# vladiant/CascadeClassifier

Hardware: AMD Instinct MI355X
Metric: detection Mwindows/sec (1080p, haarcascade_frontalface) + achieved HBM GB/s (higher is better)
Workload: dtype i32+f32 (f64 stage sums)

## Files before the change

### cascadeclassifier_amd/csrc/cc_detect.hip

```cpp
#include <hip/hip_runtime.h>

#include <algorithm>
#include <chrono>
#include <cmath>
#include <cstdlib>
#include <cstring>
#include <functional>
#include <sstream>
#include <future>
#include <memory>
#include <thread>

#include <dlfcn.h>
#include <sys/stat.h>
#include <unistd.h>

#include <atomic>
#include <map>
#include <mutex>
#include <unordered_set>

#include "cc_internal.h"

namespace ccamd {
// ... 729 lines not shown
  }
};

}

using namespace ccamd;

constexpr int kStageSlots = 3;

struct SpecCode {
  std::vector<char> code;
  int only_step = 0;
  int tile_y = TILE_Y;
};

struct cc_detector {
  Cascade m;
  unsigned long long serial = 0;
  int device = 0;
  int max_batch = 1;
  int pass_capacity = 1;
  hipStream_t own_stream = nullptr, stream = nullptr;
  DevBuf<int> d_stage_ntrees, d_stage_first;
  DevBuf<int> d_group_first;
  int n_groups = 0;
  int dense_from = 0x7fffffff;
  DevBuf<float> d_stage_thr;
  int wave_below = 0;
  int last_call_graph = 0;
  int stop_after = -1;
  int split_stumps = 0;
  DevBuf<HaarStumpDev> d_haar1, d_haar2;
  DevBuf<HaarStumpDev> d_haar1w, d_haar2w;
  DevBuf<HaarStumpDev> d_haar_g;
  DevBuf<LbpStumpDev> d_lbp_g, d_lbp16;
  int lbp16_all = 0;
  DevBuf<LbpStumpDev> d_lbp1, d_lbp2;
  DevBuf<HaarNodeDev> d_hnode1, d_hnode2;
  DevBuf<LbpNodeDev> d_lnode1, d_lnode2;
  DevBuf<int> d_tree_root, d_tree_leaf0;
  DevBuf<float> d_leaves;
  size_t lds = 0;
  size_t lds_spec = 0;
  size_t lds_extra = 0;
  int spec_tmode = 0;
  int spec_tile_y = TILE_Y;
  DevBuf<HaarStumpP16> d_haar_p16, d_haar_p16w;
  std::vector<std::unique_ptr<Plan>> plans;
  DevBuf<uint8_t> d_frames, d_pyr;
  DevBuf<int32_t> d_integ[2], d_hbuf, d_diag, d_tseg;
  hipStream_t front_stream = nullptr;
  hipEvent_t front_done[2] = {nullptr, nullptr}, eval_done[2] = {nullptr, nullptr}, batch_begin = nullptr;
  bool eval_pending[2] = {false, false};
  int overlap_front = 1;
  hipModule_t spec_mod = nullptr;
  hipFunction_t spec_fn = nullptr;
  hipModule_t spec_mod1 = nullptr;
  hipFunction_t spec_fn1 = nullptr;
  size_t lds_spec1 = 0;
  int spec_tile_y1 = TILE_Y;
  int last_stamp_tiles = 0;
  int spec_only_step = 0;
  int spec_stages = 0;
  std::thread spec_thread;
  std::atomic<int> spec_bg_state{0};
  std::vector<SpecCode> spec_bg_code;
  int spec_bg_stages = 0;
  int spec_bg_tmode = 0;
  std::string spec_bg_error;
  DevBuf<unsigned long long> d_masks[2];
  DevBuf<CandRaw> d_cands[2];
  DevBuf<CandOut> d_out[2];
  DevBuf<int> d_counts[2];
  int* h_counts = nullptr;
  uint8_t* h_frame = nullptr;
  size_t h_frame_bytes = 0;
  uint8_t* h_stage = nullptr;
  size_t h_stage_bytes = 0;
  int stage_slot = 0;
  int use_graph = 1;
// ... 121 lines not shown
    const int fi = m.stump_feature[i];
    d.nrect = 2;
    for (int j = 0; j < 3; j++) {
      const int32_t* r = &m.haar_rects[(size_t)fi * 12 + j * 4];
      const float wt = m.haar_weights[(size_t)fi * 3 + j];
      d.w[j] = wt;
      const bool used = j < 2 || wt != 0.0f;
      if (j == 2 && wt != 0.0f) d.nrect = 3;
      const int x = used ? r[0] : 0, y = used ? r[1] : 0, rw = used ? r[2] : 0, rh = used ? r[3] : 0;
      if (!m.haar_tilted[fi]) {
        d.ofs[j][0] = at(y, x);
        d.ofs[j][1] = at(y, x + rw);
        d.ofs[j][2] = at(y + rh, x);
        d.ofs[j][3] = at(y + rh, x + rw);
      } else {
        d.ofs[j][0] = tilt_shift + at(y, x);
        d.ofs[j][1] = tilt_shift + at(y + rh, x - rh);
        d.ofs[j][2] = tilt_shift + at(y + rw, x + rw);
        d.ofs[j][3] = tilt_shift + at(y + rw + rh, x + rw - rh);
      }
    }
    d.thr = m.stump_threshold[i];
    d.left = m.stump_left[i];
    d.right = m.stump_right[i];
    d.pad = (int)i;
  }
}
template <int STEP>
static void build_haar_stumps(const Cascade& m, std::vector<HaarStumpDev>& out) {
  const TileGeom<STEP> G(m.win_w, m.win_h);
  build_haar_stumps_at(m, out, [&](int y, int x) { return G.at(y, x); }, tile_words_padded(G.words()));
}
static int window_xy(int y, int x) { return (y << 16) | x; }
static void build_haar_gstumps(const Cascade& m, std::vector<HaarStumpDev>& out) { build_haar_stumps_at(m, out, window_xy, 0); }

struct SpecStump {
  std::string loads;
  std::string decls;
  std::string compute;
  double base = 0.;
  long long base_q = 0;
};

static const char* spec_stage_inline_attr() {
  const char* e = std::getenv("CCAMD_SPEC_NOINLINE");
  return (e && std::atoi(e) != 0) ? "__noinline__" : "__forceinline__";
}

static int spec_prefetch_depth(int d = 2) {
  if (const char* e = std::getenv("CCAMD_SPEC_PREFETCH")) d = std::max(0, std::min(4, std::atoi(e)));
  return d;
}

static void spec_emit_stage(std::string& o, const std::vector<SpecStump>& st, int depth, bool parts, const std::vector<std::string>& accs,
                            bool fixed_point = false) {
  const int nt = (int)st.size();
  static const char* kSB = "      __builtin_amdgcn_sched_barrier(0);\n";
  for (const SpecStump& t : st) o += "      " + t.decls + "\n";
  const int P = parts ? SPEC_PARTS : 1;
  char buf[128];
  int prev_nonempty = -1;
  for (int k = 0; k < P; k++) {
    const int e0 = (int)((long long)k * nt / P), e1 = (int)((long long)(k + 1) * nt / P);
    if (e0 == e1) continue;
    if (parts)
      snprintf(buf, sizeof(buf), "      if (p_lo > %d && p_lo <= %d) {\n", prev_nonempty, k);
    else
// ... 29 lines not shown
    }
    o += "      }\n";
  }
}

static std::string spec_stage_source_lbp(const Cascade& m, int n_stages, bool tile16);
template <int STEP>
static void build_lbp_stumps(const Cascade& m, std::vector<LbpStumpDev>& out);
static void build_lbp_stumps16(const Cascade& m, std::vector<LbpStumpDev>& out);

enum { TILE_32 = 0, TILE_16 = 1, TILE_PAIR16 = 2 };

static bool fits16(long long area) { return 255LL * area <= 65535LL; }

static std::vector<std::array<int, 4>> pieces16(int x, int y, int w, int h) {
  std::vector<std::array<int, 4>> out;
  const bool along_x = w >= h;
  const int len = along_x ? w : h;
  for (int k = 1; k <= std::max(len, 1); k++) {
    out.clear();
    bool ok = true;
    for (int i = 0; i < k; i++) {
      const int a = (int)((long long)i * len / k), b = (int)((long long)(i + 1) * len / k);
      if (a == b) continue;
      const std::array<int, 4> pc = along_x ? std::array<int, 4>{x + a, y, b - a, h} : std::array<int, 4>{x, y + a, w, b - a};
      ok = ok && fits16((long long)pc[2] * pc[3]);
      out.push_back(pc);
    }
    if (ok) return out;
  }
  return {};
}

static bool tile16_eligible(const Cascade& m, int n_stages) {
  if (m.max_nodes_per_tree > 1) return false;
  const int total = (int)m.stage_ntrees.size();
  n_stages = std::min<int>(n_stages, total);
  const char* on = std::getenv("CCAMD_SPEC_TILE16");
  if (on ? std::atoi(on) == 0 : !(m.feature_type == CC_FEATURE_LBP && n_stages == total)) return false;
  if (m.feature_type == CC_FEATURE_HAAR) {
    if (m.has_tilted) return false;
    const int nrx = m.win_w - 2, nry = m.win_h - 2;
    if (nrx < 2 || !fits16((long long)(nrx - (nrx >> 1)) * nry)) return false;
    if (!fits16(std::max(m.win_w, m.win_h))) return false;
    return true;
  }
  for (int s = 0; s < n_stages; s++)
    for (int i = 0; i < m.stage_ntrees[(size_t)s]; i++) {
      const int32_t* r = &m.lbp_rects[(size_t)m.stump_feature[(size_t)m.stage_first[(size_t)s] + i] * 4];
      if (!fits16((long long)r[2] * r[3])) return false;
    }
  return true;
}

static bool build_haar_stumps_p16(const Cascade& m, std::vector<HaarStumpP16>& out) {
  const TileGeomP G(m.win_w, m.win_h);
  out.assign(m.stump_feature.size(), HaarStumpP16{});
  for (size_t i = 0; i < out.size(); i++) {
    HaarStumpP16& d = out[i];
    std::memset(&d, 0, sizeof(d));
    const int fi = m.stump_feature[i];
    if (m.haar_tilted[(size_t)fi]) return false;
    d.nrect = 2;
    int np = 0;
    for (int j = 0; j < 3; j++) {
      const int32_t* r = &m.haar_rects[(size_t)fi * 12 + j * 4];
      const float wt = m.haar_weights[(size_t)fi * 3 + j];
      d.w[j] = wt;
      const bool used = j < 2 || wt != 0.0f;
      if (j == 2 && wt != 0.0f) d.nrect = 3;
      if (!used || r[2] <= 0 || r[3] <= 0) continue;
      const auto pcs = pieces16(r[0], r[1], r[2], r[3]);
      if (pcs.empty()) return false;
      for (const auto& pc : pcs) {
        if (np >= P16_PIECES) return false;
        const int o4[4] = {G.at(pc[1], pc[0]), G.at(pc[1], pc[0] + pc[2]), G.at(pc[1] + pc[3], pc[0]), G.at(pc[1] + pc[3], pc[0] + pc[2])};
        for (int k = 0; k < 4; k++) {
          if (o4[k] < 0 || o4[k] > 65535) return false;
// ... 1049 lines not shown
    };
    EvalLaunch launches[2];
    int n_launches = 0;
    const bool run_spec = d->spec_fn && d->m.max_nodes_per_tree <= 1;
    if (run_spec) {
      const int want[2][2] = {{d->spec_tile_y, d->spec_only_step}, {d->spec_fn1 ? d->spec_tile_y1 : 0, 1}};
      for (int i = 0; i < 2; i++) {
        if (want[i][0] == 0) continue;
        EvalLaunch L{i == 0 ? d->spec_fn : d->spec_fn1, i == 0 ? d->lds_spec : d->lds_spec1, P->n_tiles, P->d_tiles.p};
        if (!(want[i][0] == TILE_Y && want[i][1] == 0)) {
          const auto it = P->other_tiles.find(tile_list_key(want[i][0], want[i][1]));
          if (it == P->other_tiles.end() || !it->second)
            return set_error(CC_ERR_HIP, "internal: no tile list for tiles of %d window rows (step %d)", want[i][0], want[i][1]);
          L.n_tiles = it->second->n;
          L.tiles = it->second->d.p;
        }
        launches[n_launches++] = L;
      }
    } else
      launches[n_launches++] = EvalLaunch{nullptr, d->lds, P->n_tiles, P->d_tiles.p};
    size_t stamp_tiles = 0;
    for (int i = 0; i < n_launches; i++) stamp_tiles += (size_t)launches[i].n_tiles;
    if (std::getenv("CCAMD_DEBUG_STAMPS")) {
      CC_HIP(d->d_stamps.ensure(std::max<size_t>(stamp_tiles * (size_t)nf * STAMP_SLOTS, 1)));
      CC_HIP(hipMemsetAsync(d->d_stamps.p, 0, stamp_tiles * (size_t)nf * STAMP_SLOTS * sizeof(unsigned long long), st));
      A.stamps = d->d_stamps.p;
    }
    A.dbg_codes = debug ? d->d_dbg_codes.p : nullptr;
    A.dbg_sums = debug ? d->d_dbg_sums.p : nullptr;
    A.stumps1 = haar ? (const void*)d->d_haar1.p : (const void*)d->d_lbp1.p;
    A.stumps2 = haar ? (const void*)d->d_haar2.p : (const void*)d->d_lbp2.p;
    A.wstumps1 = d->d_haar1w.p ? (const void*)d->d_haar1w.p : A.stumps1;
    A.wstumps2 = d->d_haar2w.p ? (const void*)d->d_haar2w.p : A.stumps2;
    A.gstumps = haar ? (const void*)d->d_haar_g.p : (const void*)d->d_lbp_g.p;
    A.lbp16_all = d->lbp16_all;
    if (!haar && d->d_lbp16.p) A.wstumps2 = d->d_lbp16.p;
    if (d->spec_fn && d->spec_tmode == TILE_PAIR16) {
      A.gstumps = d->d_haar_p16.p;
      A.wstumps2 = d->d_haar_p16w.p;
    }
    A.trees = d->m.max_nodes_per_tree > 1 ? 1 : 0;
    A.nodes1 = haar ? (const void*)d->d_hnode1.p : (const void*)d->d_lnode1.p;
    A.nodes2 = haar ? (const void*)d->d_hnode2.p : (const void*)d->d_lnode2.p;
    A.tree_root = d->d_tree_root.p;
    A.tree_leaf0 = d->d_tree_leaf0.p;
    A.leaves = d->d_leaves.p;
    for (int i = 0; i < n_launches; i++) {
      const EvalLaunch& L = launches[i];
      if (L.n_tiles == 0) continue;
      A.tiles = L.tiles;
      if (L.fn) {
        void* params[] = {&A};
        EvScope ev1(d, i == 1 ? EV_EVAL_STEP1 : -1, st);
        CC_HIP(hipModuleLaunchKernel(L.fn, (unsigned)L.n_tiles, (unsigned)nf, 1, EVAL_THREADS, 1, 1, (unsigned)L.lds, st, params, nullptr));
      } else if (haar)
        hipLaunchKernelGGL(k_eval_haar, dim3(L.n_tiles, nf), dim3(EVAL_THREADS), L.lds, st, A);
      else
        hipLaunchKernelGGL(k_eval_lbp, dim3(L.n_tiles, nf), dim3(EVAL_THREADS), L.lds, st, A);
      if (A.stamps) A.stamps += (size_t)L.n_tiles * (size_t)nf * STAMP_SLOTS;
    }
    d->last_stamp_tiles = (int)stamp_tiles;
  }
  if (fs != st) {
    CC_HIP(hipEventRecord(d->eval_done[slot], st));
    d->eval_pending[slot] = true;
  }
  {
    EvScope ev(d, EV_FILTER, st);
    hipLaunchKernelGGL(k_filter_candidates, dim3(64), dim3(256), 0, st, d->d_cands[slot].p, d->d_counts[slot].p, d->cand_cap, P->d_sd.p,
                       d->d_masks[slot].p, P->mask_frame_words, d->d_out[slot].p, d->d_counts[slot].p + 1);
    if (debug && P->n_grid_rows)
      hipLaunchKernelGGL(k_debug_visited, dim3(P->n_grid_rows), dim3(256), 0, st, P->d_sd.p, ns, P->d_gridrow_first.p,
// ... 482 lines not shown
      api.lib = dlopen(name, RTLD_NOW | RTLD_LOCAL);
      if (api.lib) break;
    }
    if (!api.lib) return;
    auto sym = [&](const char* n) { return dlsym(api.lib, n); };
    api.create = reinterpret_cast<decltype(api.create)>(sym("hiprtcCreateProgram"));
    api.compile = reinterpret_cast<decltype(api.compile)>(sym("hiprtcCompileProgram"));
    api.log_size = reinterpret_cast<decltype(api.log_size)>(sym("hiprtcGetProgramLogSize"));
    api.log = reinterpret_cast<decltype(api.log)>(sym("hiprtcGetProgramLog"));
    api.code_size = reinterpret_cast<decltype(api.code_size)>(sym("hiprtcGetCodeSize"));
    api.code = reinterpret_cast<decltype(api.code)>(sym("hiprtcGetCode"));
    api.destroy = reinterpret_cast<decltype(api.destroy)>(sym("hiprtcDestroyProgram"));
    api.version = reinterpret_cast<decltype(api.version)>(sym("hiprtcVersion"));
  });
  return api;
}

static const char kSpecPrelude[] =
    "typedef signed char int8_t;\ntypedef unsigned char uint8_t;\ntypedef short int16_t;\ntypedef unsigned short uint16_t;\n"
    "typedef int int32_t;\ntypedef unsigned int uint32_t;\ntypedef long long int64_t;\ntypedef unsigned long long uint64_t;\n";

struct SpecModulePlan {
  int only_step, tile_y;
};
static std::vector<SpecModulePlan> spec_modules(const Cascade& m, int tmode) {
  auto valid = [&](int ty) { return ty >= EVAL_WAVES && ty <= 32 && ty % EVAL_WAVES == 0; };
  auto env_rows = [&](const char* name, int dflt) {
    const char* e = std::getenv(name);
    const int v = e ? std::atoi(e) : dflt;
    return valid(v) ? v : dflt;
  };
  if (tmode == TILE_PAIR16 || m.has_tilted) return {{0, TILE_Y}};
  const bool lbp16 = m.feature_type == CC_FEATURE_LBP && tmode == TILE_16;
  const bool haar32 = tmode == TILE_32 && m.feature_type == CC_FEATURE_HAAR;
  const bool rows_given = std::getenv("CCAMD_SPEC_TILE_Y") != nullptr;
  const int all = env_rows("CCAMD_SPEC_TILE_Y", lbp16 ? 20 : TILE_Y);
  const bool two = (haar32 || std::getenv("CCAMD_SPEC_TWO_MODULES")) && !std::getenv("CCAMD_SPEC_ONE_MODULE");
  if (!two) return {{0, all}};
  return {{2, env_rows("CCAMD_SPEC_TILE_Y2", all)}, {1, env_rows("CCAMD_SPEC_TILE_Y1", (haar32 && !rows_given) ? 12 : all)}};
}

static cc_status compile_specialised(const std::string& src, const std::string& arch, int n_stages, bool lbp, int tmode, int tile_y, int only_step, int win_w, int win_h, std::vector<char>& code) {
  const bool tile16 = tmode == TILE_16;
  static std::mutex mu;
  static std::map<std::string, std::vector<char>> cache;
  const std::string o_arch = "--offload-arch=" + arch, o_k = "-DCC_SPEC_STAGES=" + std::to_string(n_stages);
  const std::string o_ty = "-DCC_TILE_Y=" + std::to_string(tile_y), o_th = "-DCC_EVAL_THREADS=" + std::to_string(EVAL_THREADS);
  std::string o_w = "-DCC_EVAL_MIN_WAVES_PER_EU=" + std::to_string(tile16 ? (tile_y >= 20 ? 6 : 7) : CC_EVAL_MIN_WAVES_PER_EU);
  const std::string o_step = "-DCC_ONLY_STEP=" + std::to_string(only_step);
  if (const char* e = std::getenv("CCAMD_SPEC_WAVES_PER_EU")) o_w = "-DCC_EVAL_MIN_WAVES_PER_EU=" + std::to_string(std::max(1, std::min(8, std::atoi(e))));
  const std::string o_w0 = "-DCC_SPEC_W0=" + std::to_string(win_w), o_h0 = "-DCC_SPEC_H0=" + std::to_string(win_h);
  std::vector<const char*> optv = {o_arch.c_str(), "-O3", "-std=c++17", "-ffp-contract=off", "-fno-fast-math", o_k.c_str(), o_ty.c_str(), o_th.c_str(), o_w.c_str(), o_w0.c_str(), o_h0.c_str()};
  if (only_step) optv.push_back(o_step.c_str());
  if (lbp) optv.push_back("-DCC_SPEC_LBP");
  if (tile16) optv.push_back("-DCC_SPEC_TILE16");
  if (tmode == TILE_PAIR16) optv.push_back("-DCC_SPEC_PAIR16");
  std::vector<std::string> extra;
  if (const char* e = std::getenv("CCAMD_SPEC_EXTRA_FLAGS")) {
    std::istringstream is(e);
    for (std::string w; is >> w;) extra.push_back(w);
  }
  for (const std::string& w : extra) optv.push_back(w.c_str());
  const char* const* opts = optv.data();
  const int n_opts = (int)optv.size();
  std::string key;
  {
    int major = 0, minor = 0;
    const HipRtcApi& rtc = hiprtc_api();
    if (rtc.version) (void)rtc.version(&major, &minor);
    key += "hiprtc " + std::to_string(major) + "." + std::to_string(minor) + " ";
  }
  for (int i = 0; i < n_opts; i++) key += std::string(opts[i]) + " ";
  key += "#" + src;
  {
    std::lock_guard<std::mutex> lk(mu);
    auto it = cache.find(key);
    if (it != cache.end()) {
      code = it->second;
      return CC_OK;
    }
  }
// ... 131 lines not shown
  struct Loaded {
    hipModule_t mod = nullptr;
    hipFunction_t fn = nullptr;
    size_t lds = 0;
    int tile_y = TILE_Y, only_step = 0;
  };
  std::vector<Loaded> L;
  auto unload_all = [&]() {
    for (Loaded& x : L)
      if (x.mod) (void)hipModuleUnload(x.mod);
  };
  for (const SpecCode& c : codes) {
    Loaded x;
    x.tile_y = c.tile_y;
    x.only_step = c.only_step;
    const char* entry = c.only_step == 1 ? "k_eval_spec_step1" : c.only_step == 2 ? "k_eval_spec_step2" : "k_eval_spec";
    if (hipModuleLoadData(&x.mod, c.code.data()) != hipSuccess || hipModuleGetFunction(&x.fn, x.mod, entry) != hipSuccess) {
      (void)hipGetLastError();
      if (x.mod) (void)hipModuleUnload(x.mod);
      unload_all();
      return set_error(CC_ERR_HIP, "cc_detector_specialize: the compiled module does not load or has no entry point");
    }
    const int ty = c.tile_y;
    const int step = c.only_step ? c.only_step : debug_only_step();
    x.lds = d->lds;
    if (tmode == TILE_32) {
      const TileGeom<1> G1(d->m.win_w, d->m.win_h, ty);
      const TileGeom<2> G2(d->m.win_w, d->m.win_h, ty);
      const int words = step == 1 ? G1.words() : step == 2 ? G2.words() : std::max(G1.words(), G2.words());
      x.lds = eval_lds_bytes(words, d->m.has_tilted, haar_k, ty) + d->lds_extra;
    } else if (tmode == TILE_16) {
      const TileGeom<1> G1(d->m.win_w, d->m.win_h, ty);
      const TileGeom16 G2(d->m.win_w, d->m.win_h, ty);
      x.lds = eval_lds_bytes(std::max(G1.words(), G2.words()), false, haar_k, ty) + d->lds_extra;
    } else if (tmode == TILE_PAIR16) {
      const TileGeom<1> G1(d->m.win_w, d->m.win_h);
      const TileGeomP G2(d->m.win_w, d->m.win_h);
      x.lds = std::max(eval_lds_bytes(G1.words(), false), eval_lds_bytes_pair(G2.words())) + d->lds_extra;
      if (!d->d_haar_p16.p) {
        std::vector<HaarStumpP16> tp, tw;
        build_haar_stumps_p16(d->m, tp);
        std::vector<HaarStumpDev> geo;
        build_haar_stumps_at(d->m, geo, [&](int y, int x2) { return G2.at(y, x2); }, 0);
        const std::vector<HaarStumpDev> order = d->wave_below > 0 && !std::getenv("CCAMD_NO_WAVE_SCHEDULE") ? schedule_for_wave_phase(d->m, geo) : geo;
        tw.reserve(order.size());
        for (const HaarStumpDev& r : order) tw.push_back(tp[(size_t)r.pad]);
        CC_HIP(d->d_haar_p16.upload(tp, d->stream));
        CC_HIP(d->d_haar_p16w.upload(tw, d->stream));
        CC_HIP(hipStreamSynchronize(d->stream));
      }
    }
    if (x.lds > 64 * 1024) {
      const hipError_t e = hipFuncSetAttribute(reinterpret_cast<const void*>(x.fn), hipFuncAttributeMaxDynamicSharedMemorySize, (int)x.lds);
      if (e != hipSuccess) {
        (void)hipGetLastError();
        (void)hipModuleUnload(x.mod);
        unload_all();
        return set_error(CC_ERR_UNSUPPORTED, "cc_detector_specialize: %zu bytes of LDS per tile cannot be requested for a run-time module (%s)",
                         x.lds, hipGetErrorString(e));
      }
    }
    if (std::getenv("CCAMD_TRACE_HOST")) {
      int nb = 0;
      if (hipModuleOccupancyMaxActiveBlocksPerMultiprocessor(&nb, x.fn, EVAL_THREADS, x.lds) != hipSuccess) (void)hipGetLastError();
      std::fprintf(stderr, "[ccamd host] specialised kernel: tile mode %d, tiles of step %d (0 = all), %d window rows, %zu bytes of LDS per block, %d resident blocks per CU\n",
                   tmode, c.only_step, ty, x.lds, nb);
    }
// ... 208 lines not shown
    d->dense_from = 0x7fffffff;
    if (dense_stage >= 1)
      for (int g = (int)gf.size() - 2; g >= 1; g--)
        if (gf[(size_t)g] >= dense_stage) d->dense_from = g;
    CC_HIP(d->d_group_first.upload(gf, d->stream));
    CC_HIP(hipStreamSynchronize(d->stream));
  }
  if (trees) {
    std::vector<int> root(d->m.tree_first_node.begin(), d->m.tree_first_node.end()), leaf0(d->m.tree_first_leaf.begin(), d->m.tree_first_leaf.end());
    CC_HIP(d->d_tree_root.upload(root, d->stream));
    CC_HIP(d->d_tree_leaf0.upload(leaf0, d->stream));
    CC_HIP(d->d_leaves.upload(d->m.leaves, d->stream));
    if (haar) {
      std::vector<HaarNodeDev> n1, n2;
      build_haar_nodes<1>(d->m, n1);
      build_haar_nodes<2>(d->m, n2);
      CC_HIP(d->d_hnode1.upload(n1, d->stream));
      CC_HIP(d->d_hnode2.upload(n2, d->stream));
      CC_HIP(hipStreamSynchronize(d->stream));
    } else {
      std::vector<LbpNodeDev> n1, n2;
      build_lbp_nodes<1>(d->m, n1);
      build_lbp_nodes<2>(d->m, n2);
      CC_HIP(d->d_lnode1.upload(n1, d->stream));
      CC_HIP(d->d_lnode2.upload(n2, d->stream));
      CC_HIP(hipStreamSynchronize(d->stream));
    }
  } else if (haar) {
    std::vector<HaarStumpDev> s1, s2;
    build_haar_stumps<1>(d->m, s1);
    build_haar_stumps<2>(d->m, s2);
    CC_HIP(d->d_haar1.upload(s1, d->stream));
    CC_HIP(d->d_haar2.upload(s2, d->stream));
    std::vector<HaarStumpDev> sg;
    if (!d->m.has_tilted) build_haar_gstumps(d->m, sg);
    CC_HIP(d->d_haar_g.upload(sg, d->stream));
    CC_HIP(hipStreamSynchronize(d->stream));
    if (d->wave_below > 0 && !std::getenv("CCAMD_NO_WAVE_SCHEDULE")) {
      const std::vector<HaarStumpDev> w1 = schedule_for_wave_phase(d->m, s1), w2 = schedule_for_wave_phase(d->m, s2);
      CC_HIP(d->d_haar1w.upload(w1, d->stream));
      CC_HIP(d->d_haar2w.upload(w2, d->stream));
      CC_HIP(hipStreamSynchronize(d->stream));
    }
    CC_HIP(hipStreamSynchronize(d->stream));
  } else {
    std::vector<LbpStumpDev> s1, s2;
    build_lbp_stumps<1>(d->m, s1);
    build_lbp_stumps<2>(d->m, s2);
    CC_HIP(d->d_lbp1.upload(s1, d->stream));
    CC_HIP(d->d_lbp2.upload(s2, d->stream));
    std::vector<LbpStumpDev> sg, s16;
    build_lbp_gstumps(d->m, sg);
    CC_HIP(d->d_lbp_g.upload(sg, d->stream));
    d->lbp16_all = 1;
    for (size_t i = 0; i < d->m.stump_feature.size(); i++) {
      const int32_t* r = &d->m.lbp_rects[(size_t)d->m.stump_feature[i] * 4];
      if (!fits16((long long)r[2] * r[3])) d->lbp16_all = 0;
    }
    if (d->lbp16_all) {
      build_lbp_stumps16(d->m, s16);
      CC_HIP(d->d_lbp16.upload(s16, d->stream));
    }
    CC_HIP(hipStreamSynchronize(d->stream));
  }
  if (const char* e = std::getenv("CCAMD_AUTO_SPECIALIZE")) {
    const int k = std::atoi(e);
    if (k > 0 && d->m.max_nodes_per_tree == 1) (void)spec_start_background(d.get(), k);
  }
  *out = d.release();
// ... 867 lines not shown
```

### cascadeclassifier_amd/csrc/cc_eval_kernel.inc

```

#define CC_CONST __attribute__((address_space(4)))
template <class T>
__device__ __forceinline__ const T CC_CONST* as_const_table(const T* p) {
  return (const T CC_CONST*)p;
}
template <class T>
__device__ __forceinline__ T load_record(const T CC_CONST* p) {
  static_assert(sizeof(T) % 4 == 0, "table records are dword multiples");
  T out;
  const int CC_CONST* w = (const int CC_CONST*)p;
  int* o = reinterpret_cast<int*>(&out);
#pragma unroll
  for (unsigned i = 0; i < sizeof(T) / 4; i++) o[i] = w[i];
  return out;
}

constexpr int TILE_X = 64;
#ifndef CC_TILE_Y
#define CC_TILE_Y 8
#endif
#ifndef CC_EVAL_THREADS
#define CC_EVAL_THREADS 256
#endif
#ifndef CC_EVAL_MIN_WAVES_PER_EU
// ... 84 lines not shown
    row_stride = rs16 / 2;
  }
  __host__ __device__ int at(int r, int c) const { return r * rs16 + c; }
  __host__ __device__ int words() const { return rows * row_stride; }
};

struct TileGeomP {
  static constexpr bool k16 = false;
  int cols, rows, plane, row_stride, wrow;
  __host__ __device__ TileGeomP(int W0, int H0) {
    cols = (TILE_X - 1) * 2 + W0 + 1;
    rows = (TILE_Y - 1) * 2 + H0 + 1;
    plane = ((cols + 3) / 4 * 4) / 2;
    row_stride = 2 * plane;
    for (;; row_stride += 2) {
      const int k = (2 * row_stride + 1) & 31;
      if (k == 21 || k == 25 || k == 9 || k == 13 || k == 5) break;
    }
    wrow = 2 * row_stride + 1;
  }
  __host__ __device__ int at(int r, int c) const { return r * row_stride + (r >> 1) + (c & 1) * plane + (c >> 1); }
  __host__ __device__ int words() const { return rows * row_stride + (rows >> 1) + 2; }
};

constexpr int P16_PIECES = 6;
struct HaarStumpP16 {
  unsigned short ofs[P16_PIECES][4];
  float w[3];
  float thr, left, right;
  unsigned char rect_of[P16_PIECES];
  unsigned char npieces, nrect;
};
static_assert(sizeof(HaarStumpP16) == 80, "HaarStumpP16 is loaded dword by dword");

constexpr int TILE_WINDOWS = TILE_X * TILE_Y;
constexpr int MAX_STAGES = 64;
constexpr int PART_DOUBLES = (EVAL_WAVES - 1) * 64;
constexpr int QUEUE_ROWS = TILE_WINDOWS / 32;
constexpr int VNF_PITCH = TILE_X + 32;
__host__ __device__ inline int tile_words_padded(int tile_words) { return (tile_words + 3) & ~3; }
__host__ __device__ inline size_t eval_lds_bytes(int tile_words, bool tilted, bool haar = true, int tile_y = TILE_Y) {
  return (size_t)tile_words_padded(tile_words) * 4 * (tilted ? 2 : 1) + PART_DOUBLES * 8 + (haar ? tile_y * VNF_PITCH * 4 : 0) +
         2 * (tile_y * TILE_X) * 2 + 3 * 32 * 4;
}
constexpr int PAIR_PART = EVAL_THREADS / 2;
__host__ __device__ inline size_t eval_lds_bytes_pair(int tile_words) {
  return eval_lds_bytes(tile_words, false) - PART_DOUBLES * 8 + 2 * PAIR_PART * 8;
}

constexpr int STAGE_ROWS = 12;
template <int STEP, class Geom>
__device__ __forceinline__ void stage_tile(int32_t* lds, const Geom& G, const int32_t* __restrict__ sum,
                                           const ScaleDev& S, int x0, int y0) {
  const int lane = threadIdx.x & 63, wave = __builtin_amdgcn_readfirstlane(threadIdx.x >> 6);
  const int quads = (G.cols + 3) >> 2;
  const bool right_edge = x0 + quads * 4 - 1 > S.w;
  for (int q0 = 0; q0 < quads; q0 += 64) {
    const int qd = q0 + lane;
    const int c = qd * 4, gc = x0 + c;
    const bool in_tile = qd < quads;
    const bool col_ok = in_tile && gc <= S.w;
    for (int rb = wave; rb < G.rows; rb += EVAL_WAVES * STAGE_ROWS) {
      int4 v[STAGE_ROWS];
#pragma unroll
      for (int k = 0; k < STAGE_ROWS; k++) {
        const int r = rb + k * EVAL_WAVES, gr = y0 + r;
// ... 70 lines not shown
constexpr int STAMP_SLOTS = 40;

struct LdsReader {
  const int32_t* b;
  __device__ __forceinline__ int operator()(int ofs) const { return b[ofs]; }
};
struct GlobalReader {
  const int32_t* g;
  unsigned org;
  int pitch;
  __device__ __forceinline__ int operator()(int p) const { return g[org + (unsigned)((p >> 16) * pitch + (p & 0xffff))]; }
};
template <class R>
__device__ __forceinline__ double stump_vote(const R& rd, const HaarStumpDev& sp, float vnf) {
  const int r0 = rd(sp.ofs[0][0]) - rd(sp.ofs[0][1]) - rd(sp.ofs[0][2]) + rd(sp.ofs[0][3]);
  const int r1 = rd(sp.ofs[1][0]) - rd(sp.ofs[1][1]) - rd(sp.ofs[1][2]) + rd(sp.ofs[1][3]);
  float v = sp.w[0] * (float)r0 + sp.w[1] * (float)r1;
  if (sp.nrect == 3) {
    const int r2 = rd(sp.ofs[2][0]) - rd(sp.ofs[2][1]) - rd(sp.ofs[2][2]) + rd(sp.ofs[2][3]);
    v += sp.w[2] * (float)r2;
  }
  v *= vnf;
  return (double)(v < sp.thr ? sp.left : sp.right);
}
template <class R>
__device__ __forceinline__ double stump_vote(const R& rd, const HaarStumpDev CC_CONST* spp, float vnf) {
  return stump_vote(rd, load_record(spp), vnf);
}

struct Lds16Reader {
  const unsigned short* h;
  __device__ __forceinline__ int operator()(int ofs) const { return (int)h[ofs]; }
};
template <bool M16, class R>
__device__ __forceinline__ float lbp_vote_f(const R& rd, const LbpStumpDev& sp) {
  int p[16];
#pragma unroll
  for (int j = 0; j < 16; j++) p[j] = rd(sp.ofs[j]);
  auto cell = [&](int a, int b, int c2, int d) {
    const int v = p[a] - p[b] - p[c2] + p[d];
    return M16 ? (v & 0xffff) : v;
  };
  const int c = cell(5, 6, 9, 10);
  const bool b7 = cell(0, 1, 4, 5) >= c, b6 = cell(1, 2, 5, 6) >= c, b5 = cell(2, 3, 6, 7) >= c;
  const int lo = (cell(6, 7, 10, 11) >= c ? 16 : 0) | (cell(10, 11, 14, 15) >= c ? 8 : 0) | (cell(9, 10, 13, 14) >= c ? 4 : 0) |
                 (cell(8, 9, 12, 13) >= c ? 2 : 0) | (cell(4, 5, 8, 9) >= c ? 1 : 0);
  const int l0 = b5 ? sp.subset[1] : sp.subset[0], l1 = b5 ? sp.subset[3] : sp.subset[2], l2 = b5 ? sp.subset[5] : sp.subset[4],
            l3 = b5 ? sp.subset[7] : sp.subset[6];
  const int m0 = b6 ? l1 : l0, m1 = b6 ? l3 : l2;
  const unsigned w = (unsigned)(b7 ? m1 : m0);
  return ((w >> lo) & 1u) ? sp.left : sp.right;
}

template <class R>
__device__ __forceinline__ double stump_vote(const R& rd, const LbpStumpDev CC_CONST* sp, float) {
  int p[16];
#pragma unroll
  for (int j = 0; j < 16; j++) p[j] = rd(sp->ofs[j]);
  const int c = p[5] - p[6] - p[9] + p[10];
  const int lbp = (p[0] - p[1] - p[4] + p[5] >= c ? 128 : 0) | (p[1] - p[2] - p[5] + p[6] >= c ? 64 : 0) |
                  (p[2] - p[3] - p[6] + p[7] >= c ? 32 : 0) | (p[6] - p[7] - p[10] + p[11] >= c ? 16 : 0) |
                  (p[10] - p[11] - p[14] + p[15] >= c ? 8 : 0) | (p[9] - p[10] - p[13] + p[14] >= c ? 4 : 0) |
                  (p[8] - p[9] - p[12] + p[13] >= c ? 2 : 0) | (p[4] - p[5] - p[8] + p[9] >= c ? 1 : 0);
  const int word = sp->subset[lbp >> 5];
  return (double)((word & (1 << (lbp & 31))) ? sp->left : sp->right);
}
// ... 105 lines not shown
struct cc_select {
  using type = A;
};
template <class A, class B>
struct cc_select<false, A, B> {
  using type = B;
};

template <int STEP, bool HAAR, bool TREES>
__device__ __forceinline__ void eval_tile(const EvalArgs& A, int32_t* lds, const int4 T, const ScaleDev& S) {
  using Stump = typename cc_select<HAAR, HaarStumpDev, LbpStumpDev>::type;
  using Node = typename cc_select<HAAR, HaarNodeDev, LbpNodeDev>::type;
  const Node* __restrict__ nodes = reinterpret_cast<const Node*>(STEP == 2 ? A.nodes2 : A.nodes1);
#ifdef CC_SPEC_W0
  constexpr int W0 = CC_SPEC_W0, H0 = CC_SPEC_H0;
#else
  const int W0 = A.W0, H0 = A.H0;
#endif
#ifdef CC_SPEC_TILE16
  constexpr bool G16 = STEP == 2 && !TREES;
#else
  constexpr bool G16 = false;
#endif
  using Geom = typename cc_select<G16, TileGeom16, TileGeom<STEP>>::type;
  const Geom G(W0, H0);
  double* s_part = reinterpret_cast<double*>(lds + tile_words_padded(G.words()) * ((HAAR && A.tilt_chan >= 0) ? 2 : 1));
  float* s_vnf = reinterpret_cast<float*>(s_part + PART_DOUBLES);
  unsigned short* s_q = reinterpret_cast<unsigned short*>(s_vnf + (HAAR ? TILE_Y * VNF_PITCH : 0));
  int* s_cnt = reinterpret_cast<int*>(s_q + 2 * TILE_WINDOWS);
  const int frame = blockIdx.y;
  const int32_t* sum = A.integ + ((size_t)frame * A.nchan + 0) * A.int_frame_elems + S.int_ofs;
  const int lane = threadIdx.x & 63, wave = __builtin_amdgcn_readfirstlane(threadIdx.x >> 6);
  const int gx0 = T.y * TILE_X, gy0 = T.z * TILE_Y;
  const Stump CC_CONST* stumps = as_const_table(reinterpret_cast<const Stump*>(G16 ? A.gstumps : STEP == 2 ? A.stumps2 : A.stumps1));
  const int CC_CONST* stage_first = as_const_table(A.stage_first);
  const int CC_CONST* stage_ntrees = as_const_table(A.stage_ntrees);
  const float CC_CONST* stage_thr = as_const_table(A.stage_thr);
  const bool dbg = A.dbg_codes != nullptr && frame == 0;
  auto stamp = [&](int slot) {
    if (A.stamps && threadIdx.x == 0)
      A.stamps[((size_t)blockIdx.y * gridDim.x + blockIdx.x) * STAMP_SLOTS + slot] = __builtin_amdgcn_s_memtime();
  };
  stamp(0);

  unsigned sq_raw[WIN_PER_THREAD][4];
#pragma unroll
  for (int k = 0; k < WIN_PER_THREAD; k++) {
    sq_raw[k][0] = sq_raw[k][1] = sq_raw[k][2] = sq_raw[k][3] = 0;
    if (HAAR) {
      const int gx = min(gx0 + lane, S.nx - 1), gy = min(gy0 + wave * WIN_PER_THREAD + k, S.ny - 1);
      {
        const unsigned* sq = reinterpret_cast<const unsigned*>(A.integ + ((size_t)frame * A.nchan + 1) * A.int_frame_elems + S.int_ofs);
        const int nrx = W0 - 2, nry = H0 - 2;
        size_t q0;
        int dx;
        if (STEP == 2 && A.sq_compact) {
          q0 = (size_t)(gy * 2 + 1) * S.pitchI + gx;
          dx = nrx >> 1;
        } else {
          q0 = (size_t)(gy * STEP + 1) * S.pitchI + (gx * STEP + 1);
          dx = nrx;
        }
        sq_raw[k][0] = sq[q0];
        sq_raw[k][1] = sq[q0 + dx];
        sq_raw[k][2] = sq[q0 + (size_t)nry * S.pitchI];
        sq_raw[k][3] = sq[q0 + (size_t)nry * S.pitchI + dx];
      }
    }
  }
#ifdef CC_PRIO_STAGE
  __builtin_amdgcn_s_setprio(CC_PRIO_STAGE);
#endif
  stage_tile<STEP>(lds, G, sum, S, gx0 * STEP, gy0 * STEP);
  if (HAAR && A.tilt_chan >= 0)
    stage_tile<STEP>(lds + tile_words_padded(G.words()), G,
                     A.integ + ((size_t)frame * A.nchan + A.tilt_chan) * A.int_frame_elems + S.int_ofs, S, gx0 * STEP, gy0 * STEP);
  if (threadIdx.x < 3 * 32) s_cnt[threadIdx.x] = 0;
  unsigned valsq_pre[WIN_PER_THREAD];
#pragma unroll
  for (int k = 0; k < WIN_PER_THREAD; k++) valsq_pre[k] = sq_raw[k][0] - sq_raw[k][1] - sq_raw[k][2] + sq_raw[k][3];
  __syncthreads();
#ifdef CC_PRIO_STAGE
  __builtin_amdgcn_s_setprio(0);
#endif
  stamp(1);

  if (A.stop_after == -2) return;
  auto window_base = [&](int id) { return ((id >> 6) * STEP) * G.row_stride + (id & 63); };
  auto table_reader = [&](int id) {
    if constexpr (G16)
      return GlobalReader{sum, (unsigned)((gy0 + (id >> 6)) * STEP) * (unsigned)S.pitchI + (unsigned)((gx0 + (id & 63)) * STEP), S.pitchI};
    else
      return LdsReader{lds + window_base(id)};
  };
  auto report = [&](int id, int code, double last) {
    const size_t o = (size_t)S.win_ofs + (size_t)(gy0 + (id >> 6)) * S.nx + (gx0 + (id & 63));
    A.dbg_codes[o] = code;
    if (A.dbg_sums) A.dbg_sums[o] = last;
  };
  auto emit_candidate = [&](int id, double last_sum) {
    const int slot = atomicAdd(A.cand_count, 1);
    if (slot < A.cand_cap) A.cands[slot] = CandRaw{frame, T.x, gx0 + (id & 63), gy0 + (id >> 6), last_sum};
  };
  const int skew = (STEP * G.row_stride) & 31;
  auto win_class = [&](int id) { return ((id & 63) + skew * (id >> 6)) & 31; };
  auto vnf_slot = [&](int id) { return (id >> 6) * (TILE_X + skew) + (id & 63); };
  auto enqueue = [&](bool pass, int id, int g) {
    if (g >= A.dense_from) {
      const unsigned long long m = __ballot(pass);
      int first = 0;
      if (lane == 0 && m) first = atomicAdd(&s_cnt[(g % 3) * 32], __builtin_popcountll(m));
      first = __builtin_amdgcn_readfirstlane(first);
      if (pass) s_q[(g & 1) * TILE_WINDOWS + first + __builtin_amdgcn_mbcnt_hi((unsigned)(m >> 32), __builtin_amdgcn_mbcnt_lo((unsigned)m, 0))] = (unsigned short)id;
    } else if (pass) {
      const int c = win_class(id);
      const int row = atomicAdd(&s_cnt[(g % 3) * 32 + c], 1);
      s_q[(g & 1) * TILE_WINDOWS + row * 32 + c] = (unsigned short)id;
    }
  };

  const int CC_CONST* group_first = as_const_table(A.group_first);
  auto stage_sum = [&](int s, int id, const int32_t* b, float vnf, bool want) -> double {
    double acc = 0.;
    const int first = stage_first[s], nt = stage_ntrees[s];
    if constexpr (TREES) {
      for (int j = 0; j < nt; j++) {
        const int root = as_const_table(A.tree_root)[first + j], leaf0 = as_const_table(A.tree_leaf0)[first + j];
        if (want) acc += tree_vote(b, nodes, root, leaf0, A.leaves, vnf);
      }
    } else {
#ifdef CC_SPEC_STAGES
      if (s < CC_SPEC_STAGES) return spec_stage<STEP>(s, 0, SPEC_PARTS, b, vnf);
#endif
      const auto rd = table_reader(id);
      if constexpr (HAAR) {
        Stump cur = load_record(stumps + first);
        for (int j = 0; j < nt; j++) {
          const Stump nxt = load_record(stumps + first + min(j + 1, nt - 1));
          acc += stump_vote(rd, cur, vnf);
          cur = nxt;
        }
      } else {
        for (int j = 0; j < nt; j++) acc += stump_vote(rd, stumps + first + j, vnf);
      }
    }
    return acc;
  };

  if constexpr (!HAAR && !TREES && WIN_PER_THREAD > 2) {
    const int gx = gx0 + lane;
    const double thr0 = (double)stage_thr[0];
    const int nt0 = stage_ntrees[0];
#pragma unroll 1
    for (int k = 0; k < WIN_PER_THREAD; k++) {
      const int ly = wave * WIN_PER_THREAD + k;
      const int gy = gy0 + ly;
      const int id = ly * 64 + lane;
      const int32_t* b = lds + (ly * STEP) * G.row_stride + lane;
      const bool alive = gx < S.nx && gy < S.ny;
      double acc = 0.;
      if (__any(alive)) {
#ifdef CC_SPEC_STAGES
        acc = spec_stage<STEP>(0, 0, SPEC_PARTS, b, 1.f);
#else
        for (int i = 0; i < nt0; i++) acc += stump_vote(LdsReader{b}, stumps + i, 1.f);
#endif
      }
      (void)nt0;
      bool pass = alive && !(acc < thr0);
      const bool rej0 = alive && !pass;
      const unsigned long long m = __ballot(rej0);
// ... 221 lines not shown
        } else
          enqueue(alive, id, qg + 1);
      }
    }
    auto finish = [&](bool valid, int id, double acc) {
      const bool pass = valid && !(acc < thr);
      if (dbg && valid && !pass) report(id, -st, acc);
      if (last_group) {
        if (pass) {
          emit_candidate(id, acc);
          if (dbg) report(id, 1, acc);
        }
      } else
        enqueue(pass, id, qg + 1);
    };
    if (ns > 1) {
      const int slice = wave % ns, grp = wave / ns;
      const int row = (g_split + grp) * 2 + half;
      const int i = grp * 64 + lane;
      const bool valid = row < my_rows;
      const int id = valid ? q[min(row, QUEUE_ROWS - 1) * 32 + cls] : cls;
      double acc = 0.;
      if (grp < rem) {
        [[maybe_unused]] const int32_t* b = lds + window_base(id);
        const float vnf = HAAR ? s_vnf[vnf_slot(id)] : 1.f;
        [[maybe_unused]] const auto rd = table_reader(id);
        if constexpr (HAAR) {
#ifdef CC_SPEC_STAGES
          if (!TREES && st < CC_SPEC_STAGES) {
            acc = spec_stage<STEP>(st, slice * (SPEC_PARTS / ns), (slice + 1) * (SPEC_PARTS / ns), b, vnf);
          } else
#endif
          if (slice < nt) {
            Stump cur = load_record(stumps + first + slice);
            for (int j = slice; j < nt; j += ns) {
              const Stump nxt = load_record(stumps + first + min(j + ns, nt - 1));
              acc += stump_vote(rd, cur, vnf);
              cur = nxt;
            }
          }
        } else {
#ifdef CC_SPEC_STAGES
          if (!TREES && st < CC_SPEC_STAGES)
            acc = spec_stage<STEP>(st, slice * (SPEC_PARTS / ns), (slice + 1) * (SPEC_PARTS / ns), b, vnf);
          else
#endif
            for (int j = slice; j < nt; j += ns) acc += stump_vote(rd, stumps + first + j, vnf);
        }
        if (slice) s_part[(slice - 1) * (EVAL_THREADS / ns) + i] = acc;
      }
      __syncthreads();
      if (grp < rem && slice == 0) {
        for (int k = 1; k < ns; k++) acc += s_part[(k - 1) * (EVAL_THREADS / ns) + i];
        finish(valid, id, acc);
      }
    }
  }
  if (qg >= A.ngroups || n == 0) {
    stamp(STAMP_SLOTS - 1);
    return;
  }

  if constexpr (HAAR && !TREES) {
    const unsigned short* q = s_q + (qg & 1) * TILE_WINDOWS;
    const Stump* wstumps = reinterpret_cast<const Stump*>(G16 ? A.gstumps : STEP == 2 ? A.wstumps2 : A.wstumps1);
    unsigned short* my_list = reinterpret_cast<unsigned short*>(s_part) + wave * 64;
    int numbered = 0;
    for (int r0 = 0; r0 < rows; r0 += 2) {
      const int row = r0 + half;
      const bool valid = row < my_rows;
      const int id = valid ? q[row * 32 + cls] : 0;
      const unsigned long long mask = __ballot(valid);
      const int number = numbered + __builtin_amdgcn_mbcnt_hi((unsigned)(mask >> 32), __builtin_amdgcn_mbcnt_lo((unsigned)mask, 0));
      if (valid && number % EVAL_WAVES == wave) my_list[number / EVAL_WAVES] = (unsigned short)id;
      numbered += __builtin_popcountll(mask);
    }
    const int cnt = (numbered - wave + EVAL_WAVES - 1) / EVAL_WAVES;
    const int my_id = lane < cnt ? my_list[lane] : 0;
    unsigned long long alive = cnt >= 64 ? ~0ull : ((1ull << cnt) - 1ull);
    const bool w_stamps = st + 2 < 30;
    if (w_stamps) stamp(30);
    double tot = 0., last = 0.;
    int rej = 0;
    int s2 = st;
    for (; s2 < A.nstages && alive; s2++) {
      if (A.stop_after >= 0 && s2 > A.stop_after) break;
      const int first = stage_first[s2], nt = stage_ntrees[s2];
      for (int c = 0; c < nt; c += 64) {
        const int j = c + lane;
        const Stump rec = wstumps[first + min(j, nt - 1)];
        for (unsigned long long m = alive; m; m &= m - 1ull) {
          const int k = __builtin_ctzll(m);
          const int id = __builtin_amdgcn_readlane(my_id, k);
          const float vnf = s_vnf[vnf_slot(id)];
          const double part = j < nt ? stump_vote(table_reader(id), rec, vnf) : 0.;
          const double total = wave_sum_f64(part);
          if (lane == k) tot += total;
        }
      }
      const bool mine = (alive >> lane) & 1ull;
      const bool pass = mine && !(tot < (double)stage_thr[s2]);
      if (mine) {
        last = tot;
        if (!pass) rej = s2;
      }
      tot = 0.;
      alive = __ballot(pass);
      if (w_stamps && s2 - st < 8) stamp(31 + s2 - st);
    }
    const bool accepted = s2 == A.nstages && ((alive >> lane) & 1ull);
    if (lane < cnt) {
      if (accepted) emit_candidate(my_id, last);
      if (dbg && (accepted || !((alive >> lane) & 1ull))) report(my_id, accepted ? 1 : -rej, last);
    }
  }
  if constexpr (!HAAR && !TREES && EVAL_WAVES >= 4) {
    const unsigned short* q = s_q + (qg & 1) * TILE_WINDOWS;
    unsigned short* my_list = reinterpret_cast<unsigned short*>(s_part) + wave * 64;
    float* votes = reinterpret_cast<float*>(reinterpret_cast<char*>(s_part) + EVAL_WAVES * 128) + wave * 64;
    int numbered = 0;
    for (int r0 = 0; r0 < rows; r0 += 2) {
      const int row = r0 + half;
      const bool valid = row < my_rows;
// ... 566 lines not shown
```

Measured before the change: 18240.

## Use 16-bit LDS integral tile for Haar step-2 specialised evaluation

Enables the 16-bit tile mode by default for Haar cascades. It adds a compact HaarStump16 record with ushort offsets, splitting rectangles into pieces whose sums fit 16 bits and recombining them modulo 2^16. The step-2 kernel then reads the integral image from LDS as 16-bit values, where it previously read 32-bit values or went to global memory. This halves LDS per tile and allows more waves per EU, with per-module tile rows and wave counts tuned. The cost is extra piece arithmetic for rectangles that have to be split, a more complex setup, and removal of the global Haar stump path.

```diff
diff --git a/cascadeclassifier_amd/csrc/cc_detect.hip b/cascadeclassifier_amd/csrc/cc_detect.hip
--- a/cascadeclassifier_amd/csrc/cc_detect.hip
+++ b/cascadeclassifier_amd/csrc/cc_detect.hip
@@ -785,7 +785,6 @@
   int split_stumps = 0;
   DevBuf<HaarStumpDev> d_haar1, d_haar2;
   DevBuf<HaarStumpDev> d_haar1w, d_haar2w;
-  DevBuf<HaarStumpDev> d_haar_g;
   DevBuf<LbpStumpDev> d_lbp_g, d_lbp16;
   int lbp16_all = 0;
   DevBuf<LbpStumpDev> d_lbp1, d_lbp2;
@@ -799,6 +798,7 @@
   int spec_tmode = 0;
   int spec_tile_y = TILE_Y;
   DevBuf<HaarStumpP16> d_haar_p16, d_haar_p16w;
+  DevBuf<HaarStump16> d_haar16, d_haar16w;
   std::vector<std::unique_ptr<Plan>> plans;
   DevBuf<uint8_t> d_frames, d_pyr;
   DevBuf<int32_t> d_integ[2], d_hbuf, d_diag, d_tseg;
@@ -986,7 +986,6 @@
   build_haar_stumps_at(m, out, [&](int y, int x) { return G.at(y, x); }, tile_words_padded(G.words()));
 }
 static int window_xy(int y, int x) { return (y << 16) | x; }
-static void build_haar_gstumps(const Cascade& m, std::vector<HaarStumpDev>& out) { build_haar_stumps_at(m, out, window_xy, 0); }
 
 struct SpecStump {
   std::string loads;
@@ -1082,18 +1081,61 @@
   return {};
 }
 
+static bool build_haar_stumps16(const Cascade& m, std::vector<HaarStump16>& out) {
+  const TileGeom16 G(m.win_w, m.win_h);
+  out.assign(m.stump_feature.size(), HaarStump16{});
+  for (size_t i = 0; i < out.size(); i++) {
+    HaarStump16& d = out[i];
+    std::memset(&d, 0, sizeof(d));
+    const int fi = m.stump_feature[i];
+    if (m.haar_tilted[(size_t)fi]) return false;
+    d.nrect = 2;
+    int nx = 0;
+    for (int j = 0; j < 3; j++) {
+      const int32_t* r = &m.haar_rects[(size_t)fi * 12 + j * 4];
+      const float wt = m.haar_weights[(size_t)fi * 3 + j];
+      d.w[j] = wt;
+      const bool used = j < 2 || wt != 0.0f;
+      if (j == 2 && wt != 0.0f) d.nrect = 3;
+      if (!used || r[2] <= 0 || r[3] <= 0) continue;
+      const auto pcs = pieces16(r[0], r[1], r[2], r[3]);
+      if (pcs.empty()) return false;
+      for (size_t q = 0; q < pcs.size(); q++) {
+        const auto& pc = pcs[q];
+        const int slot = q == 0 ? j : 3 + nx;
+        if (q > 0) {
+          if (nx >= S16_EXTRA) return false;
+          d.xrect = (unsigned char)(d.xrect | (j << (2 * nx)));
+          nx++;
+        }
+        const int o4[4] = {G.at(pc[1], pc[0]), G.at(pc[1], pc[0] + pc[2]), G.at(pc[1] + pc[3], pc[0]), G.at(pc[1] + pc[3], pc[0] + pc[2])};
+        for (int k = 0; k < 4; k++) {
+          if (o4[k] < 0 || o4[k] > 65535) return false;
+          d.ofs[slot][k] = (unsigned short)o4[k];
+        }
+      }
+    }
+    d.nextra = (unsigned char)nx;
+    d.thr = m.stump_threshold[i];
+    d.left = m.stump_left[i];
+    d.right = m.stump_right[i];
+  }
+  return true;
+}
+
 static bool tile16_eligible(const Cascade& m, int n_stages) {
   if (m.max_nodes_per_tree > 1) return false;
   const int total = (int)m.stage_ntrees.size();
   n_stages = std::min<int>(n_stages, total);
   const char* on = std::getenv("CCAMD_SPEC_TILE16");
-  if (on ? std::atoi(on) == 0 : !(m.feature_type == CC_FEATURE_LBP && n_stages == total)) return false;
+  if (on ? std::atoi(on) == 0 : !(m.feature_type == CC_FEATURE_HAAR || n_stages == total)) return false;
   if (m.feature_type == CC_FEATURE_HAAR) {
     if (m.has_tilted) return false;
     const int nrx = m.win_w - 2, nry = m.win_h - 2;
     if (nrx < 2 || !fits16((long long)(nrx - (nrx >> 1)) * nry)) return false;
     if (!fits16(std::max(m.win_w, m.win_h))) return false;
-    return true;
+    std::vector<HaarStump16> tmp;
+    return build_haar_stumps16(m, tmp);
   }
   for (int s = 0; s < n_stages; s++)
     for (int i = 0; i < m.stage_ntrees[(size_t)s]; i++) {
@@ -2209,12 +2251,16 @@
     A.stumps2 = haar ? (const void*)d->d_haar2.p : (const void*)d->d_lbp2.p;
     A.wstumps1 = d->d_haar1w.p ? (const void*)d->d_haar1w.p : A.stumps1;
     A.wstumps2 = d->d_haar2w.p ? (const void*)d->d_haar2w.p : A.stumps2;
-    A.gstumps = haar ? (const void*)d->d_haar_g.p : (const void*)d->d_lbp_g.p;
+    A.gstumps = haar ? nullptr : (const void*)d->d_lbp_g.p;
     A.lbp16_all = d->lbp16_all;
     if (!haar && d->d_lbp16.p) A.wstumps2 = d->d_lbp16.p;
     if (d->spec_fn && d->spec_tmode == TILE_PAIR16) {
       A.gstumps = d->d_haar_p16.p;
       A.wstumps2 = d->d_haar_p16w.p;
+    }
+    if (haar && d->spec_fn && d->spec_tmode == TILE_16) {
+      A.gstumps = d->d_haar16.p;
+      A.wstumps2 = d->d_haar16w.p;
     }
     A.trees = d->m.max_nodes_per_tree > 1 ? 1 : 0;
     A.nodes1 = haar ? (const void*)d->d_hnode1.p : (const void*)d->d_lnode1.p;
@@ -2763,12 +2809,14 @@
   };
   if (tmode == TILE_PAIR16 || m.has_tilted) return {{0, TILE_Y}};
   const bool lbp16 = m.feature_type == CC_FEATURE_LBP && tmode == TILE_16;
-  const bool haar32 = tmode == TILE_32 && m.feature_type == CC_FEATURE_HAAR;
+  const bool haar = m.feature_type == CC_FEATURE_HAAR;
   const bool rows_given = std::getenv("CCAMD_SPEC_TILE_Y") != nullptr;
   const int all = env_rows("CCAMD_SPEC_TILE_Y", lbp16 ? 20 : TILE_Y);
-  const bool two = (haar32 || std::getenv("CCAMD_SPEC_TWO_MODULES")) && !std::getenv("CCAMD_SPEC_ONE_MODULE");
+  const bool two = (haar || std::getenv("CCAMD_SPEC_TWO_MODULES")) && !std::getenv("CCAMD_SPEC_ONE_MODULE");
   if (!two) return {{0, all}};
-  return {{2, env_rows("CCAMD_SPEC_TILE_Y2", all)}, {1, env_rows("CCAMD_SPEC_TILE_Y1", (haar32 && !rows_given) ? 12 : all)}};
+  const bool haar16 = haar && tmode == TILE_16;
+  return {{2, env_rows("CCAMD_SPEC_TILE_Y2", (haar16 && !rows_given) ? 12 : all)},
+          {1, env_rows("CCAMD_SPEC_TILE_Y1", (haar && !rows_given) ? 12 : all)}};
 }
 
 static cc_status compile_specialised(const std::string& src, const std::string& arch, int n_stages, bool lbp, int tmode, int tile_y, int only_step, int win_w, int win_h, std::vector<char>& code) {
@@ -2777,7 +2825,11 @@
   static std::map<std::string, std::vector<char>> cache;
   const std::string o_arch = "--offload-arch=" + arch, o_k = "-DCC_SPEC_STAGES=" + std::to_string(n_stages);
   const std::string o_ty = "-DCC_TILE_Y=" + std::to_string(tile_y), o_th = "-DCC_EVAL_THREADS=" + std::to_string(EVAL_THREADS);
-  std::string o_w = "-DCC_EVAL_MIN_WAVES_PER_EU=" + std::to_string(tile16 ? (tile_y >= 20 ? 6 : 7) : CC_EVAL_MIN_WAVES_PER_EU);
+  int waves = tile16 ? (tile_y >= 20 ? 6 : 7) : CC_EVAL_MIN_WAVES_PER_EU;
+  if (tile16 && !lbp && only_step == 1) waves = CC_EVAL_MIN_WAVES_PER_EU;
+  if (tile16 && !lbp && only_step == 2)
+    waves = std::max(1, std::min(8, (int)((160 * 1024) / eval_lds_bytes(TileGeom16(win_w, win_h, tile_y).words(), false, true, tile_y))));
+  std::string o_w = "-DCC_EVAL_MIN_WAVES_PER_EU=" + std::to_string(waves);
   const std::string o_step = "-DCC_ONLY_STEP=" + std::to_string(only_step);
   if (const char* e = std::getenv("CCAMD_SPEC_WAVES_PER_EU")) o_w = "-DCC_EVAL_MIN_WAVES_PER_EU=" + std::to_string(std::max(1, std::min(8, std::atoi(e))));
   const std::string o_w0 = "-DCC_SPEC_W0=" + std::to_string(win_w), o_h0 = "-DCC_SPEC_H0=" + std::to_string(win_h);
@@ -2975,7 +3027,37 @@
     } else if (tmode == TILE_16) {
       const TileGeom<1> G1(d->m.win_w, d->m.win_h, ty);
       const TileGeom16 G2(d->m.win_w, d->m.win_h, ty);
-      x.lds = eval_lds_bytes(std::max(G1.words(), G2.words()), false, haar_k, ty) + d->lds_extra;
+      const int words = step == 1 ? G1.words() : step == 2 ? G2.words() : std::max(G1.words(), G2.words());
+      x.lds = eval_lds_bytes(words, false, haar_k, ty) + d->lds_extra;
+      if (haar_k && !d->d_haar16.p) {
+        std::vector<HaarStump16> tp, tw;
+        if (!build_haar_stumps16(d->m, tp)) {
+          unload_all();
+          (void)hipModuleUnload(x.mod);
+          return set_error(CC_ERR_HIP, "cc_detector_specialize: a stump does not fit the 16-bit tile's record");
+        }
+        std::vector<HaarStumpDev> g0, geo;
+        build_haar_stumps_at(d->m, g0, [&](int y, int x2) { return G2.at(y, x2) >> 1; }, 0);
+        Cascade parts = d->m;
+        parts.stage_first.clear();
+        parts.stage_ntrees.clear();
+        for (size_t s = 0; s < d->m.stage_ntrees.size(); s++) {
+          const int first = d->m.stage_first[s], nt = d->m.stage_ntrees[s];
+          for (int extra = 0; extra < 2; extra++) {
+            const int f = (int)geo.size();
+            for (int i = first; i < first + nt; i++)
+              if ((tp[(size_t)i].nextra > 0) == (extra == 1)) geo.push_back(g0[(size_t)i]);
+            parts.stage_first.push_back(f);
+            parts.stage_ntrees.push_back((int)geo.size() - f);
+          }
+        }
+        const std::vector<HaarStumpDev> order = d->wave_below > 0 && !std::getenv("CCAMD_NO_WAVE_SCHEDULE") ? schedule_for_wave_phase(parts, geo) : geo;
+        tw.reserve(order.size());
+        for (const HaarStumpDev& r : order) tw.push_back(tp[(size_t)r.pad]);
+        CC_HIP(d->d_haar16.upload(tp, d->stream));
+        CC_HIP(d->d_haar16w.upload(tw, d->stream));
+        CC_HIP(hipStreamSynchronize(d->stream));
+      }
     } else if (tmode == TILE_PAIR16) {
       const TileGeom<1> G1(d->m.win_w, d->m.win_h);
       const TileGeomP G2(d->m.win_w, d->m.win_h);
@@ -3250,9 +3332,6 @@
     build_haar_stumps<2>(d->m, s2);
     CC_HIP(d->d_haar1.upload(s1, d->stream));
     CC_HIP(d->d_haar2.upload(s2, d->stream));
-    std::vector<HaarStumpDev> sg;
-    if (!d->m.has_tilted) build_haar_gstumps(d->m, sg);
-    CC_HIP(d->d_haar_g.upload(sg, d->stream));
     CC_HIP(hipStreamSynchronize(d->stream));
     if (d->wave_below > 0 && !std::getenv("CCAMD_NO_WAVE_SCHEDULE")) {
       const std::vector<HaarStumpDev> w1 = schedule_for_wave_phase(d->m, s1), w2 = schedule_for_wave_phase(d->m, s2);
diff --git a/cascadeclassifier_amd/csrc/cc_eval_kernel.inc b/cascadeclassifier_amd/csrc/cc_eval_kernel.inc
--- a/cascadeclassifier_amd/csrc/cc_eval_kernel.inc
+++ b/cascadeclassifier_amd/csrc/cc_eval_kernel.inc
@@ -140,6 +140,15 @@
   unsigned char npieces, nrect;
 };
 static_assert(sizeof(HaarStumpP16) == 80, "HaarStumpP16 is loaded dword by dword");
+
+constexpr int S16_EXTRA = P16_PIECES - 3;
+struct HaarStump16 {
+  unsigned short ofs[P16_PIECES][4];
+  float w[3];
+  float thr, left, right;
+  unsigned char nrect, nextra, xrect, pad;
+};
+static_assert(sizeof(HaarStump16) == 76, "HaarStump16 is loaded dword by dword");
 
 constexpr int TILE_WINDOWS = TILE_X * TILE_Y;
 constexpr int MAX_STAGES = 64;
@@ -276,6 +285,30 @@
   const unsigned short* h;
   __device__ __forceinline__ int operator()(int ofs) const { return (int)h[ofs]; }
 };
+__device__ __forceinline__ double stump_vote(const Lds16Reader& rd, const HaarStump16& sp, float vnf) {
+  auto piece = [&](int p) { return (rd(sp.ofs[p][0]) - rd(sp.ofs[p][1]) - rd(sp.ofs[p][2]) + rd(sp.ofs[p][3])) & 0xffff; };
+  int r0 = piece(0), r1 = piece(1), r2 = 0;
+  if (sp.nrect == 3) r2 = piece(2);
+  if (sp.nextra) {
+#pragma unroll
+    for (int i = 0; i < S16_EXTRA; i++) {
+      if (i < sp.nextra) {
+        const int v = piece(3 + i), r = (sp.xrect >> (2 * i)) & 3;
+        r0 += r == 0 ? v : 0;
+        r1 += r == 1 ? v : 0;
+        r2 += r == 2 ? v : 0;
+      }
+    }
+  }
+  float v = sp.w[0] * (float)r0 + sp.w[1] * (float)r1;
+  if (sp.nrect == 3) v += sp.w[2] * (float)r2;
+  v *= vnf;
+  return (double)(v < sp.thr ? sp.left : sp.right);
+}
+__device__ __forceinline__ double stump_vote(const Lds16Reader& rd, const HaarStump16 CC_CONST* spp, float vnf) {
+  return stump_vote(rd, load_record(spp), vnf);
+}
+
 template <bool M16, class R>
 __device__ __forceinline__ float lbp_vote_f(const R& rd, const LbpStumpDev& sp) {
   int p[16];
@@ -447,7 +480,8 @@
   const int32_t* sum = A.integ + ((size_t)frame * A.nchan + 0) * A.int_frame_elems + S.int_ofs;
   const int lane = threadIdx.x & 63, wave = __builtin_amdgcn_readfirstlane(threadIdx.x >> 6);
   const int gx0 = T.y * TILE_X, gy0 = T.z * TILE_Y;
-  const Stump CC_CONST* stumps = as_const_table(reinterpret_cast<const Stump*>(G16 ? A.gstumps : STEP == 2 ? A.stumps2 : A.stumps1));
+  using TStump = typename cc_select<HAAR && G16, HaarStump16, Stump>::type;
+  const TStump CC_CONST* stumps = as_const_table(reinterpret_cast<const TStump*>(G16 ? A.gstumps : STEP == 2 ? A.stumps2 : A.stumps1));
   const int CC_CONST* stage_first = as_const_table(A.stage_first);
   const int CC_CONST* stage_ntrees = as_const_table(A.stage_ntrees);
   const float CC_CONST* stage_thr = as_const_table(A.stage_thr);
@@ -503,7 +537,9 @@
   if (A.stop_after == -2) return;
   auto window_base = [&](int id) { return ((id >> 6) * STEP) * G.row_stride + (id & 63); };
   auto table_reader = [&](int id) {
-    if constexpr (G16)
+    if constexpr (G16 && HAAR)
+      return Lds16Reader{reinterpret_cast<const unsigned short*>(lds + window_base(id))};
+    else if constexpr (G16)
       return GlobalReader{sum, (unsigned)((gy0 + (id >> 6)) * STEP) * (unsigned)S.pitchI + (unsigned)((gx0 + (id & 63)) * STEP), S.pitchI};
     else
       return LdsReader{lds + window_base(id)};
@@ -549,9 +585,9 @@
 #endif
       const auto rd = table_reader(id);
       if constexpr (HAAR) {
-        Stump cur = load_record(stumps + first);
+        TStump cur = load_record(stumps + first);
         for (int j = 0; j < nt; j++) {
-          const Stump nxt = load_record(stumps + first + min(j + 1, nt - 1));
+          const TStump nxt = load_record(stumps + first + min(j + 1, nt - 1));
           acc += stump_vote(rd, cur, vnf);
           cur = nxt;
         }
@@ -839,9 +875,9 @@
           } else
 #endif
           if (slice < nt) {
-            Stump cur = load_record(stumps + first + slice);
+            TStump cur = load_record(stumps + first + slice);
             for (int j = slice; j < nt; j += ns) {
-              const Stump nxt = load_record(stumps + first + min(j + ns, nt - 1));
+              const TStump nxt = load_record(stumps + first + min(j + ns, nt - 1));
               acc += stump_vote(rd, cur, vnf);
               cur = nxt;
             }
@@ -870,7 +906,7 @@
 
   if constexpr (HAAR && !TREES) {
     const unsigned short* q = s_q + (qg & 1) * TILE_WINDOWS;
-    const Stump* wstumps = reinterpret_cast<const Stump*>(G16 ? A.gstumps : STEP == 2 ? A.wstumps2 : A.wstumps1);
+    const TStump* wstumps = reinterpret_cast<const TStump*>(STEP == 2 ? A.wstumps2 : A.wstumps1);
     unsigned short* my_list = reinterpret_cast<unsigned short*>(s_part) + wave * 64;
     int numbered = 0;
     for (int r0 = 0; r0 < rows; r0 += 2) {
@@ -895,7 +931,7 @@
       const int first = stage_first[s2], nt = stage_ntrees[s2];
       for (int c = 0; c < nt; c += 64) {
         const int j = c + lane;
-        const Stump rec = wstumps[first + min(j, nt - 1)];
+        const TStump rec = wstumps[first + min(j, nt - 1)];
         for (unsigned long long m = alive; m; m &= m - 1ull) {
           const int k = __builtin_ctzll(m);
           const int id = __builtin_amdgcn_readlane(my_id, k);
```

Result: faster. 18730, median of 6 (+2.7%).
